# gusanagy/Hybrid-Diffusion-Underwater-Atmopheric-Image-Enhancement

Measured on AMD Instinct MI355X. Metric: denoising-steps/sec (256x256, T=1000), higher is better.
Workload: dtype f32 (tensors and accumulation fp32; every operand of the attention contractions as 2xfp16 pieces -- scores: a balance per product term, four terms at d_head 16 / three at d_head 32; P.V: three terms -- and of the 3x3 convs behind GroupNorm likewise (other 3x3 convs: 3xbf16 pieces), on the 16-bit MFM

## Files before the change

### hybrid-diffusion-underwater-atmopheric-image-enhancement_amd/csrc/attention_x3p.hip

```cpp
#include <stdlib.h>

#include "common.h"
#include "device.h"

using namespace hdiff;

namespace {

constexpr int D = 32;
constexpr int KT = 64;
constexpr int THREADS = 256;
constexpr int NQT = 3;

__global__ __launch_bounds__(THREADS, 2) void mha_flash_fwd_x3p_kernel(const __bf16* __restrict__ ws, float* __restrict__ out,
                                                                      float* __restrict__ lse2, int C, int L, float one) {
  constexpr int KS = D / 16;
  constexpr int KROWB = D * 2 + 16;
  constexpr int KPART = KT * KROWB;
  constexpr int VROWB = KT * 2 + 8;
  constexpr int VPART = D * VROWB;
  constexpr int NKC = NQT * KT * D / 8;
  constexpr int NVC = 2 * D * 8;
  constexpr int NLD = (NKC + NVC) / THREADS;
  static_assert((NKC + NVC) % THREADS == 0, "staging geometry");
  constexpr int QB = 256;
  constexpr int VBASE = NQT * KPART;
  constexpr int BUFB = (VBASE + 2 * VPART + 15) / 16 * 16;
  __shared__ __attribute__((aligned(16))) unsigned char smem[2][BUFB];

  const int tid = threadIdx.x, lane = tid & 63, wave = tid >> 6;
  const int l31 = lane & 31, h = lane >> 5;
  const TileId tile = xcd_tile();
  const int head = tile.head, b = tile.b;
  const int heads = gridDim.y;
  const int qblk0 = tile.x * QB + wave * 64;
  const size_t piece = (size_t)L * D;
  const __bf16* qs = ws + ((size_t)b * heads + head) * F_COUNT * piece;
  const __bf16* ks = qs + F_K * piece;
  const __bf16* vs = qs + F_V * piece;
  const int ntiles = L / KT;

  u32x4 qop[2][NQT][KS];
#pragma unroll
  for (int G = 0; G < 2; ++G) {
    const int q = qblk0 + 32 * G + l31;
#pragma unroll
    for (int p = 0; p < 2; ++p)
#pragma unroll
      for (int s = 0; s < KS; ++s)
        qop[G][p][s] = *reinterpret_cast<const u32x4*>(qs + p * piece + (size_t)q * D + 16 * s + 8 * h);
    const unsigned dn2 = PAIR_DOWN2;
#pragma unroll
    for (int s = 0; s < KS; ++s) {
      unsigned w4[4];
#pragma unroll
      for (int w = 0; w < 4; ++w) asm("v_pk_mul_f16 %0, %1, %2" : "=v"(w4[w]) : "v"(qop[G][0][s][w]), "v"(dn2));
      qop[G][2][s] = u32x4{w4[0], w4[1], w4[2], w4[3]};
    }
  }

  const unsigned char* gsrc[NLD];
  int lds_off[NLD];
  int gstep[NLD];
#pragma unroll
  for (int i = 0; i < NLD; ++i) {
    const int c = i * THREADS + tid;
    if (c < NKC) {
      const int p = c / (KT * D / 8), rem = c - p * (KT * D / 8);
      const int key = rem / (D / 8), part = rem - key * (D / 8);
      gsrc[i] = reinterpret_cast<const unsigned char*>(ks + p * piece) + (size_t)rem * 16;
      lds_off[i] = p * KPART + key * KROWB + part * 16;
      gstep[i] = KT * D * 2;
    } else {
      const int cv = c - NKC;
      const int p = cv / (D * 8), rem = cv - p * (D * 8);
      const int d = rem >> 3, seg = rem & 7;
      gsrc[i] = reinterpret_cast<const unsigned char*>(vs + p * piece + (size_t)d * L) + seg * 16;
      lds_off[i] = VBASE + p * VPART + d * VROWB + seg * 16;
      gstep[i] = KT * 2;
    }
  }
  u32x4 stage[NLD];
  auto stage_load = [&](int t) {
#pragma unroll
    for (int i = 0; i < NLD; ++i) stage[i] = *reinterpret_cast<const u32x4*>(gsrc[i] + (size_t)t * gstep[i]);
  };
  auto stage_store = [&](int buf) {
#pragma unroll
    for (int i = 0; i < NLD; ++i) {
      unsigned char* dst = &smem[buf][lds_off[i]];
      *reinterpret_cast<u32x2*>(dst) = u32x2{stage[i][0], stage[i][1]};
      *reinterpret_cast<u32x2*>(dst + 8) = u32x2{stage[i][2], stage[i][3]};
    }
  };

  const int kaddr = l31 * KROWB + 16 * h;
  int vaddr[2];
#pragma unroll
  for (int p = 0; p < 2; ++p) vaddr[p] = p * VPART + l31 * VROWB + 8 * h;

  f32x16 O[2], negm16;
  f32x2 l_run[2];
  float negm2[2] = {0.f, 0.f};
#pragma unroll
  for (int G = 0; G < 2; ++G) {
    l_run[G] = f32x2{0.f, 0.f};
#pragma unroll
    for (int r = 0; r < 16; ++r) O[G][r] = 0.f;
  }
#pragma unroll
  for (int r = 0; r < 16; ++r) negm16[r] = 0.f;

  auto load_k = [&](int buf, int kb, u32x4 (&kop)[NQT][KS]) {
    const unsigned char* kbuf = smem[buf] + kb * 32 * KROWB + kaddr;
#pragma unroll
    for (int p = 0; p < NQT; ++p)
#pragma unroll
      for (int s = 0; s < KS; ++s) kop[p][s] = *reinterpret_cast<const u32x4*>(kbuf + p * KPART + 32 * s);
  };
  auto load_v = [&](int buf, int kb, u32x4 (&vop)[2][2]) {
    const unsigned char* vbuf = smem[buf] + VBASE + kb * 64;
#pragma unroll
    for (int ab = 0; ab < 2; ++ab)
#pragma unroll
      for (int p = 0; p < 2; ++p) {
        const unsigned char* src = vbuf + vaddr[p] + 32 * ab;
        const u32x2 lo = *reinterpret_cast<const u32x2*>(src);
        const u32x2 hi2 = *reinterpret_cast<const u32x2*>(src + 16);
        vop[ab][p] = u32x4{lo[0], lo[1], hi2[0], hi2[1]};
      }
  };
  auto qk = [&](const u32x4 (&kop)[NQT][KS], int G, f32x16 c) {
    f32x16 S = c;
#pragma unroll
    for (int term = 0; term < NQT; ++term)
#pragma unroll
      for (int s = 0; s < KS; ++s) {
        u32x4 qb = qop[G][term][s];
        if ((HDIFF_MUTANT & 2) && term == 1)
#pragma unroll
          for (int w = 0; w < 4; ++w) qb[w] &= 0xffe0ffe0u;
        S = mfma_f16(kop[term][s], qb, S);
      }
    return S;
  };
  auto exp_pairs = [&](const f32x16& S, u32x4 (&pop)[2][2], float& sum0, float& sum1) {
    sum0 = 0.f; sum1 = 0.f;
#pragma unroll
    for (int j = 0; j < 4; ++j) {
      const float p0 = __builtin_amdgcn_exp2f(S[4 * j]), p1 = __builtin_amdgcn_exp2f(S[4 * j + 1]);
      const float p2 = __builtin_amdgcn_exp2f(S[4 * j + 2]), p3 = __builtin_amdgcn_exp2f(S[4 * j + 3]);
      sum0 += p0 + p2;
      sum1 += p1 + p3;
      unsigned a0, a1, c0, c1;
      split2(p0, p1, one, a0, a1);
      split2(p2, p3, one, c0, c1);
      const int ab = j >> 1, o = (j & 1) * 2;
      pop[ab][0][o] = a0; pop[ab][1][o] = a1;
      pop[ab][0][o + 1] = c0; pop[ab][1][o + 1] = c1;
    }
  };
  auto softmax_pairs = [&](f32x16& S, int G, u32x4 (&pop)[2][2]) {
    float sum0, sum1;
    exp_pairs(S, pop, sum0, sum1);
    if (__builtin_amdgcn_ballot_w64(sum0 + sum1 >= P_TRIP) != 0ull) {
      float mx = fmaxf(fmaxf(S[0], S[1]), fmaxf(S[2], S[3]));
#pragma unroll
      for (int j = 1; j < 4; ++j) mx = fmaxf(mx, fmaxf(fmaxf(S[4 * j], S[4 * j + 1]), fmaxf(S[4 * j + 2], S[4 * j + 3])));
      mx = fmaxf(mx, __shfl_xor(mx, 32, 64));
      const float delta = (mx > P_SHIFT + 1.0f) ? __builtin_ceilf(mx - P_SHIFT) : 0.f;
      const int e = -(int)delta;
#pragma unroll
      for (int r = 0; r < 16; ++r) O[G][r] = __builtin_ldexpf(O[G][r], e);
      l_run[G][0] = __builtin_ldexpf(l_run[G][0], e);
      l_run[G][1] = __builtin_ldexpf(l_run[G][1], e);
      negm2[G] -= delta;
#pragma unroll
      for (int r = 0; r < 16; ++r) S[r] -= delta;
      exp_pairs(S, pop, sum0, sum1);
    }
    l_run[G][0] += sum0;
    l_run[G][1] += sum1;
  };
  auto pv = [&](const u32x4 (&vop)[2][2], const u32x4 (&pop)[2][2], int G) {
#pragma unroll
    for (int ab = 0; ab < 2; ++ab) {
      O[G] = mfma_f16(vop[ab][1], pop[ab][0], O[G]);
      O[G] = mfma_f16(vop[ab][0], pop[ab][1], O[G]);
      O[G] = mfma_f16(vop[ab][0], pop[ab][0], O[G]);
    }
  };

  stage_load(0);
  stage_store(0);
  __syncthreads();
  stage_load(ntiles > 1 ? 1 : 0);
  {
    u32x4 K0[NQT][KS];
    load_k(0, 0, K0);
    const f32x16 s0 = qk(K0, 0, negm16), s1 = qk(K0, 1, negm16);
    float t0 = s0[0], t1 = s1[0];
#pragma unroll
    for (int r = 1; r < 16; ++r) { t0 = fmaxf(t0, s0[r]); t1 = fmaxf(t1, s1[r]); }
    negm2[0] = P_SHIFT - fmaxf(t0, __shfl_xor(t0, 32, 64));
    negm2[1] = P_SHIFT - fmaxf(t1, __shfl_xor(t1, 32, 64));
  }
  auto block = [&](int buf, int kb) {
    u32x4 kop[NQT][KS], vop[2][2];
    load_k(buf, kb, kop);
    load_v(buf, kb, vop);
    f32x16 S2[2];
#pragma unroll
    for (int G = 0; G < 2; ++G) {
      float nm = negm2[G];
      asm volatile("" : "+v"(nm));
#pragma unroll
      for (int r = 0; r < 16; ++r) negm16[r] = nm;
      S2[G] = qk(kop, G, negm16);
    }
#pragma unroll
    for (int G = 0; G < 2; ++G) {
      u32x4 pop[2][2];
      softmax_pairs(S2[G], G, pop);
      pv(vop, pop, G);
    }
  };
  block(0, 0);
  block(0, 1);
  stage_store(1);
  __syncthreads();
  for (int t = 1; t < ntiles; ++t) {
    const int buf = t & 1;
    stage_load((t + 1 < ntiles) ? t + 1 : t);
    block(buf, 0);
    block(buf, 1);
    stage_store(buf ^ 1);
    __syncthreads();
  }

  float* obase = out + ((size_t)b * C + (size_t)head * D) * L;
  const float* vinv = reinterpret_cast<const float*>(qs + 8 * piece);
#pragma unroll
  for (int G = 0; G < 2; ++G) {
    float lt = l_run[G][0] + l_run[G][1];
    lt += __shfl_xor(lt, 32, 64);
    const bool bad = !(lt < OVERFLOW_LIMIT);
    const float inv = bad ? __builtin_nanf("") : 1.0f / lt;
    const int q = qblk0 + 32 * G + l31;
    if (lse2 != nullptr && h == 0)
      lse2[((size_t)b * heads + head) * L + q] = bad ? __builtin_nanf("") : __builtin_amdgcn_logf(lt) - negm2[G];
#pragma unroll
    for (int r = 0; r < 16; ++r) {
      const int d = 8 * (r >> 2) + 4 * h + (r & 3);
      obase[(size_t)d * L + q] = (O[G][r] * inv) * vinv[d];
    }
  }
}

}

namespace hdiff {

int64_t mha_fwd_x3p_workspace(int B, int C, int heads, int L) {
  const int Dh = C / heads;
  if ((Dh != 16 && Dh != 32) || L % 256 != 0 || L < 512) return 0;
  return (int64_t)B * C * L * F_COUNT * 2 + mha_fwd_h2_tail_bytes(B, C);
}

void launch_mha_fwd_x3p(const float* qkv, float* o, float* lse2, int B, int C, int heads, int L, float qscale, void* ws,
                        hipStream_t stream) {
  launch_qk_split_h2(qkv, ws, B, C, heads, L, qscale, stream);
  launch_v_split_h2(qkv, ws, B, C, heads, L, stream);
  hipLaunchKernelGGL(mha_flash_fwd_x3p_kernel, dim3(L / 256, heads, B), dim3(THREADS), 0, stream, (const __bf16*)ws, o, lse2, C, L, 1.0f);
}

}
```

Measured before the change: 2.978.

## Software-pipeline QK/softmax/PV across query groups and DMA K tiles into LDS

The flash-attention kernel now interleaves the QK and PV MFMAs of one query group with the exp/split softmax VALU work of the other, using sched_barrier to pin the interleave. K tiles are loaded straight into LDS with a direct global-to-LDS DMA using an XOR-swizzled layout, replacing the padded register-staged copy. Prefetch moves two tiles ahead with an explicit vmcnt wait. This aims to hide MFMA and VALU latency behind each other and cut staging instructions, at the cost of more register pressure and more complex scheduling.

```diff
diff --git a/hybrid-diffusion-underwater-atmopheric-image-enhancement_amd/csrc/attention_x3p.hip b/hybrid-diffusion-underwater-atmopheric-image-enhancement_amd/csrc/attention_x3p.hip
--- a/hybrid-diffusion-underwater-atmopheric-image-enhancement_amd/csrc/attention_x3p.hip
+++ b/hybrid-diffusion-underwater-atmopheric-image-enhancement_amd/csrc/attention_x3p.hip
@@ -1,4 +1,6 @@
 #include <stdlib.h>
+
+#include <type_traits>
 
 #include "common.h"
 #include "device.h"
@@ -15,14 +17,14 @@
 __global__ __launch_bounds__(THREADS, 2) void mha_flash_fwd_x3p_kernel(const __bf16* __restrict__ ws, float* __restrict__ out,
                                                                       float* __restrict__ lse2, int C, int L, float one) {
   constexpr int KS = D / 16;
-  constexpr int KROWB = D * 2 + 16;
+  constexpr int KROWB = D * 2;
   constexpr int KPART = KT * KROWB;
   constexpr int VROWB = KT * 2 + 8;
   constexpr int VPART = D * VROWB;
-  constexpr int NKC = NQT * KT * D / 8;
   constexpr int NVC = 2 * D * 8;
-  constexpr int NLD = (NKC + NVC) / THREADS;
-  static_assert((NKC + NVC) % THREADS == 0, "staging geometry");
+  constexpr int NLD = NVC / THREADS;
+  static_assert(NVC % THREADS == 0, "staging geometry");
+  static_assert(NQT * KPART == 3 * (THREADS / 64) * 1024, "LDS-DMA geometry: twelve 1 KiB runs, three per wave");
   constexpr int QB = 256;
   constexpr int VBASE = NQT * KPART;
   constexpr int BUFB = (VBASE + 2 * VPART + 15) / 16 * 16;
@@ -59,31 +61,33 @@
     }
   }
 
+  const unsigned kdma_voff = (unsigned)(((lane >> 2) * 4 + ((lane & 3) ^ ((lane >> 4) & 3))) * 16);
+  const unsigned lds0 = (unsigned)(size_t)(lds_byte*)&smem[0][0];
+  const unsigned char* kdma = reinterpret_cast<const unsigned char*>(ks);
+  auto dma_k = [&](int t, int buf) {
+    const int w3 = __builtin_amdgcn_readfirstlane(wave) * 3;
+#pragma unroll
+    for (int i = 0; i < 3; ++i) {
+      const int run = w3 + i, p = run >> 2, quarter = run & 3;
+      const unsigned char* src = kdma + (size_t)p * (piece * 2) + (size_t)t * KPART + quarter * 1024;
+      const unsigned dst = __builtin_amdgcn_readfirstlane(lds0 + buf * BUFB + run * 1024);
+      dma_1k(src, kdma_voff, dst);
+    }
+  };
   const unsigned char* gsrc[NLD];
   int lds_off[NLD];
-  int gstep[NLD];
 #pragma unroll
   for (int i = 0; i < NLD; ++i) {
-    const int c = i * THREADS + tid;
-    if (c < NKC) {
-      const int p = c / (KT * D / 8), rem = c - p * (KT * D / 8);
-      const int key = rem / (D / 8), part = rem - key * (D / 8);
-      gsrc[i] = reinterpret_cast<const unsigned char*>(ks + p * piece) + (size_t)rem * 16;
-      lds_off[i] = p * KPART + key * KROWB + part * 16;
-      gstep[i] = KT * D * 2;
-    } else {
-      const int cv = c - NKC;
-      const int p = cv / (D * 8), rem = cv - p * (D * 8);
-      const int d = rem >> 3, seg = rem & 7;
-      gsrc[i] = reinterpret_cast<const unsigned char*>(vs + p * piece + (size_t)d * L) + seg * 16;
-      lds_off[i] = VBASE + p * VPART + d * VROWB + seg * 16;
-      gstep[i] = KT * 2;
-    }
+    const int cv = i * THREADS + tid;
+    const int p = cv / (D * 8), rem = cv - p * (D * 8);
+    const int d = rem >> 3, seg = rem & 7;
+    gsrc[i] = reinterpret_cast<const unsigned char*>(vs + p * piece + (size_t)d * L) + seg * 16;
+    lds_off[i] = VBASE + p * VPART + d * VROWB + seg * 16;
   }
   u32x4 stage[NLD];
   auto stage_load = [&](int t) {
 #pragma unroll
-    for (int i = 0; i < NLD; ++i) stage[i] = *reinterpret_cast<const u32x4*>(gsrc[i] + (size_t)t * gstep[i]);
+    for (int i = 0; i < NLD; ++i) stage[i] = *reinterpret_cast<const u32x4*>(gsrc[i] + (size_t)t * (KT * 2));
   };
   auto stage_store = [&](int buf) {
 #pragma unroll
@@ -94,31 +98,34 @@
     }
   };
 
-  const int kaddr = l31 * KROWB + 16 * h;
+  int kaddr[KS];
+#pragma unroll
+  for (int s = 0; s < KS; ++s) kaddr[s] = l31 * KROWB + 16 * ((2 * s + h) ^ ((l31 >> 2) & 3));
   int vaddr[2];
 #pragma unroll
   for (int p = 0; p < 2; ++p) vaddr[p] = p * VPART + l31 * VROWB + 8 * h;
 
-  f32x16 O[2], negm16;
+  f32x16 O[2], negm16[2];
   f32x2 l_run[2];
-  float negm2[2] = {0.f, 0.f};
 #pragma unroll
   for (int G = 0; G < 2; ++G) {
     l_run[G] = f32x2{0.f, 0.f};
 #pragma unroll
-    for (int r = 0; r < 16; ++r) O[G][r] = 0.f;
-  }
-#pragma unroll
-  for (int r = 0; r < 16; ++r) negm16[r] = 0.f;
-
-  auto load_k = [&](int buf, int kb, u32x4 (&kop)[NQT][KS]) {
-    const unsigned char* kbuf = smem[buf] + kb * 32 * KROWB + kaddr;
+    for (int r = 0; r < 16; ++r) { O[G][r] = 0.f; negm16[G][r] = 0.f; }
+  }
+
+  u32x4 kop[NQT][KS];
+  u32x4 vop[2][2];
+  f32x16 S[2];
+  u32x4 pop[2][2][2];
+  auto load_k = [&](int buf, int kb) {
+    const unsigned char* kbuf = smem[buf] + kb * 32 * KROWB;
 #pragma unroll
     for (int p = 0; p < NQT; ++p)
 #pragma unroll
-      for (int s = 0; s < KS; ++s) kop[p][s] = *reinterpret_cast<const u32x4*>(kbuf + p * KPART + 32 * s);
-  };
-  auto load_v = [&](int buf, int kb, u32x4 (&vop)[2][2]) {
+      for (int s = 0; s < KS; ++s) kop[p][s] = *reinterpret_cast<const u32x4*>(kbuf + p * KPART + kaddr[s]);
+  };
+  auto load_v = [&](int buf, int kb) {
     const unsigned char* vbuf = smem[buf] + VBASE + kb * 64;
 #pragma unroll
     for (int ab = 0; ab < 2; ++ab)
@@ -130,43 +137,82 @@
         vop[ab][p] = u32x4{lo[0], lo[1], hi2[0], hi2[1]};
       }
   };
-  auto qk = [&](const u32x4 (&kop)[NQT][KS], int G, f32x16 c) {
-    f32x16 S = c;
-#pragma unroll
-    for (int term = 0; term < NQT; ++term)
-#pragma unroll
-      for (int s = 0; s < KS; ++s) {
-        u32x4 qb = qop[G][term][s];
-        if ((HDIFF_MUTANT & 2) && term == 1)
-#pragma unroll
-          for (int w = 0; w < 4; ++w) qb[w] &= 0xffe0ffe0u;
-        S = mfma_f16(kop[term][s], qb, S);
-      }
-    return S;
-  };
-  auto exp_pairs = [&](const f32x16& S, u32x4 (&pop)[2][2], float& sum0, float& sum1) {
-    sum0 = 0.f; sum1 = 0.f;
+  constexpr int NQK = NQT * KS, NPV = 6;
+  auto qk_mfma = [&](int G, int n) {
+    const int term = n / KS, s = n - term * KS;
+    u32x4 qb = qop[G][term][s];
+    if ((HDIFF_MUTANT & 2) && term == 1)
+#pragma unroll
+      for (int w = 0; w < 4; ++w) qb[w] &= 0xffe0ffe0u;
+    S[G] = mfma_f16(kop[term][s], qb, n == 0 ? negm16[G] : S[G]);
+  };
+  auto pv_mfma = [&](int G, int n) {
+    const int ab = n / 3, term = n - ab * 3;
+    O[G] = mfma_f16(vop[ab][term == 0 ? 1 : 0], pop[G][ab][term == 1 ? 1 : 0], O[G]);
+  };
+  auto exp_pairs = [&](const f32x16& Sq, u32x4 (&pp)[2][2], float& sum0, float& sum1) {
 #pragma unroll
     for (int j = 0; j < 4; ++j) {
-      const float p0 = __builtin_amdgcn_exp2f(S[4 * j]), p1 = __builtin_amdgcn_exp2f(S[4 * j + 1]);
-      const float p2 = __builtin_amdgcn_exp2f(S[4 * j + 2]), p3 = __builtin_amdgcn_exp2f(S[4 * j + 3]);
-      sum0 += p0 + p2;
-      sum1 += p1 + p3;
+      const float p0 = __builtin_amdgcn_exp2f(Sq[4 * j]), p1 = __builtin_amdgcn_exp2f(Sq[4 * j + 1]);
+      const float p2 = __builtin_amdgcn_exp2f(Sq[4 * j + 2]), p3 = __builtin_amdgcn_exp2f(Sq[4 * j + 3]);
+      sum0 = (j == 0) ? p0 + p2 : sum0 + (p0 + p2);
+      sum1 = (j == 0) ? p1 + p3 : sum1 + (p1 + p3);
       unsigned a0, a1, c0, c1;
       split2(p0, p1, one, a0, a1);
       split2(p2, p3, one, c0, c1);
       const int ab = j >> 1, o = (j & 1) * 2;
-      pop[ab][0][o] = a0; pop[ab][1][o] = a1;
-      pop[ab][0][o + 1] = c0; pop[ab][1][o + 1] = c1;
-    }
-  };
-  auto softmax_pairs = [&](f32x16& S, int G, u32x4 (&pop)[2][2]) {
+      pp[ab][0][o] = a0; pp[ab][1][o] = a1;
+      pp[ab][0][o + 1] = c0; pp[ab][1][o + 1] = c1;
+    }
+  };
+  auto stage_fn = [&](auto g_tag, auto pend_tag, int kload_buf, int kload_kb, int vload_buf, int vload_kb) __attribute__((always_inline)) {
+    constexpr int G = decltype(g_tag)::value;
+    constexpr bool PEND = decltype(pend_tag)::value;
+    constexpr int NM = NQK + (PEND ? NPV : 0);
+    if (kload_buf >= 0) load_k(kload_buf, kload_kb);
     float sum0, sum1;
-    exp_pairs(S, pop, sum0, sum1);
+    float pe[4][4], ad[4][2];
+    unsigned u[4][2], r2[4][2];
+    _Float16 rl[4][2];
+    auto vstep = [&](int n) {
+      const int j = n / 14, r = n - j * 14;
+      if (r < 4) pe[j][r] = __builtin_amdgcn_exp2f(S[G][4 * j + r]);
+      else if (r < 6) {
+        const f16x2 p = {(_Float16)pe[j][2 * (r - 4)], (_Float16)pe[j][2 * (r - 4) + 1]};
+        unsigned w = __builtin_bit_cast(unsigned, p);
+        asm("" : "+v"(w));
+        u[j][r - 4] = w;
+      } else if (r < 8) ad[j][r - 6] = pe[j][r - 6] + pe[j][r - 6 + 2];
+      else if (r < 10) rl[j][r - 8] = (_Float16)__builtin_fmaf(pe[j][2 * (r - 8)], one, -(float)__builtin_bit_cast(f16x2, u[j][r - 8])[0]);
+      else if (r < 12) {
+        const f16x2 pr = {rl[j][r - 10],
+                          (_Float16)__builtin_fmaf(pe[j][2 * (r - 10) + 1], one, -(float)__builtin_bit_cast(f16x2, u[j][r - 10])[1])};
+        unsigned w = __builtin_bit_cast(unsigned, pr);
+        asm("" : "+v"(w));
+        r2[j][r - 10] = w;
+      } else if (r == 12) sum0 = (j == 0) ? ad[j][0] : sum0 + ad[j][0];
+      else sum1 = (j == 0) ? ad[j][1] : sum1 + ad[j][1];
+    };
+    constexpr int NV = 56;
+#pragma unroll
+    for (int i = 0; i < NM; ++i) {
+      if (PEND && i < NPV) pv_mfma(G ^ 1, i);
+      else qk_mfma(G ^ 1, i - (PEND ? NPV : 0));
+      if (PEND && i == NPV - 1 && vload_buf >= 0) load_v(vload_buf, vload_kb);
+#pragma unroll
+      for (int n = NV * i / NM; n < NV * (i + 1) / NM; ++n) vstep(n);
+      __builtin_amdgcn_sched_barrier(0);
+    }
+#pragma unroll
+    for (int j = 0; j < 4; ++j) {
+      const int ab = j >> 1, o = (j & 1) * 2;
+      pop[G][ab][0][o] = u[j][0]; pop[G][ab][1][o] = r2[j][0];
+      pop[G][ab][0][o + 1] = u[j][1]; pop[G][ab][1][o + 1] = r2[j][1];
+    }
     if (__builtin_amdgcn_ballot_w64(sum0 + sum1 >= P_TRIP) != 0ull) {
-      float mx = fmaxf(fmaxf(S[0], S[1]), fmaxf(S[2], S[3]));
-#pragma unroll
-      for (int j = 1; j < 4; ++j) mx = fmaxf(mx, fmaxf(fmaxf(S[4 * j], S[4 * j + 1]), fmaxf(S[4 * j + 2], S[4 * j + 3])));
+      float mx = fmaxf(fmaxf(S[G][0], S[G][1]), fmaxf(S[G][2], S[G][3]));
+#pragma unroll
+      for (int j = 1; j < 4; ++j) mx = fmaxf(mx, fmaxf(fmaxf(S[G][4 * j], S[G][4 * j + 1]), fmaxf(S[G][4 * j + 2], S[G][4 * j + 3])));
       mx = fmaxf(mx, __shfl_xor(mx, 32, 64));
       const float delta = (mx > P_SHIFT + 1.0f) ? __builtin_ceilf(mx - P_SHIFT) : 0.f;
       const int e = -(int)delta;
@@ -174,69 +220,57 @@
       for (int r = 0; r < 16; ++r) O[G][r] = __builtin_ldexpf(O[G][r], e);
       l_run[G][0] = __builtin_ldexpf(l_run[G][0], e);
       l_run[G][1] = __builtin_ldexpf(l_run[G][1], e);
-      negm2[G] -= delta;
-#pragma unroll
-      for (int r = 0; r < 16; ++r) S[r] -= delta;
-      exp_pairs(S, pop, sum0, sum1);
+#pragma unroll
+      for (int r = 0; r < 16; ++r) { negm16[G][r] -= delta; S[G][r] -= delta; }
+      exp_pairs(S[G], pop[G], sum0, sum1);
     }
     l_run[G][0] += sum0;
     l_run[G][1] += sum1;
   };
-  auto pv = [&](const u32x4 (&vop)[2][2], const u32x4 (&pop)[2][2], int G) {
-#pragma unroll
-    for (int ab = 0; ab < 2; ++ab) {
-      O[G] = mfma_f16(vop[ab][1], pop[ab][0], O[G]);
-      O[G] = mfma_f16(vop[ab][0], pop[ab][1], O[G]);
-      O[G] = mfma_f16(vop[ab][0], pop[ab][0], O[G]);
-    }
-  };
-
+  using G0 = std::integral_constant<int, 0>;
+  using G1 = std::integral_constant<int, 1>;
+  auto tile_fn = [&](auto first_tag, int t) __attribute__((always_inline)) {
+    constexpr bool FIRST = decltype(first_tag)::value;
+    using Pend = std::integral_constant<bool, !FIRST>;
+    const int buf = t & 1;
+    stage_fn(G0{}, Pend{}, -1, 0, FIRST ? -1 : buf, 0);
+    stage_fn(G1{}, std::true_type{}, buf, 1, -1, 0);
+    stage_fn(G0{}, std::true_type{}, -1, 0, buf, 1);
+    stage_store(buf ^ 1);
+    asm volatile("s_waitcnt vmcnt(0)" ::: "memory");
+    __syncthreads();
+    const int tn = (t + 2 < ntiles) ? t + 2 : ntiles - 1;
+    dma_k(tn, buf);
+    stage_load(tn);
+    stage_fn(G1{}, std::true_type{}, buf ^ 1, 0, -1, 0);
+  };
+
+  dma_k(0, 0);
   stage_load(0);
   stage_store(0);
+  asm volatile("s_waitcnt vmcnt(0)" ::: "memory");
   __syncthreads();
+  dma_k(ntiles > 1 ? 1 : 0, 1);
   stage_load(ntiles > 1 ? 1 : 0);
+  load_k(0, 0);
   {
-    u32x4 K0[NQT][KS];
-    load_k(0, 0, K0);
-    const f32x16 s0 = qk(K0, 0, negm16), s1 = qk(K0, 1, negm16);
-    float t0 = s0[0], t1 = s1[0];
-#pragma unroll
-    for (int r = 1; r < 16; ++r) { t0 = fmaxf(t0, s0[r]); t1 = fmaxf(t1, s1[r]); }
-    negm2[0] = P_SHIFT - fmaxf(t0, __shfl_xor(t0, 32, 64));
-    negm2[1] = P_SHIFT - fmaxf(t1, __shfl_xor(t1, 32, 64));
-  }
-  auto block = [&](int buf, int kb) {
-    u32x4 kop[NQT][KS], vop[2][2];
-    load_k(buf, kb, kop);
-    load_v(buf, kb, vop);
-    f32x16 S2[2];
-#pragma unroll
-    for (int G = 0; G < 2; ++G) {
-      float nm = negm2[G];
-      asm volatile("" : "+v"(nm));
-#pragma unroll
-      for (int r = 0; r < 16; ++r) negm16[r] = nm;
-      S2[G] = qk(kop, G, negm16);
-    }
-#pragma unroll
-    for (int G = 0; G < 2; ++G) {
-      u32x4 pop[2][2];
-      softmax_pairs(S2[G], G, pop);
-      pv(vop, pop, G);
-    }
-  };
-  block(0, 0);
-  block(0, 1);
-  stage_store(1);
-  __syncthreads();
-  for (int t = 1; t < ntiles; ++t) {
-    const int buf = t & 1;
-    stage_load((t + 1 < ntiles) ? t + 1 : t);
-    block(buf, 0);
-    block(buf, 1);
-    stage_store(buf ^ 1);
-    __syncthreads();
-  }
+#pragma unroll
+    for (int n = 0; n < NQK; ++n) { qk_mfma(0, n); qk_mfma(1, n); }
+    float t0 = S[0][0], t1 = S[1][0];
+#pragma unroll
+    for (int r = 1; r < 16; ++r) { t0 = fmaxf(t0, S[0][r]); t1 = fmaxf(t1, S[1][r]); }
+    const float nm0 = P_SHIFT - fmaxf(t0, __shfl_xor(t0, 32, 64)), nm1 = P_SHIFT - fmaxf(t1, __shfl_xor(t1, 32, 64));
+#pragma unroll
+    for (int r = 0; r < 16; ++r) { negm16[0][r] = nm0; negm16[1][r] = nm1; }
+  }
+  load_v(0, 0);
+#pragma unroll
+  for (int n = 0; n < NQK; ++n) qk_mfma(0, n);
+  tile_fn(std::true_type{}, 0);
+  for (int t = 1; t < ntiles; ++t) tile_fn(std::false_type{}, t);
+#pragma unroll
+  for (int n = 0; n < NPV; ++n) pv_mfma(1, n);
+  asm volatile("s_waitcnt vmcnt(0)" ::: "memory");
 
   float* obase = out + ((size_t)b * C + (size_t)head * D) * L;
   const float* vinv = reinterpret_cast<const float*>(qs + 8 * piece);
@@ -248,7 +282,7 @@
     const float inv = bad ? __builtin_nanf("") : 1.0f / lt;
     const int q = qblk0 + 32 * G + l31;
     if (lse2 != nullptr && h == 0)
-      lse2[((size_t)b * heads + head) * L + q] = bad ? __builtin_nanf("") : __builtin_amdgcn_logf(lt) - negm2[G];
+      lse2[((size_t)b * heads + head) * L + q] = bad ? __builtin_nanf("") : __builtin_amdgcn_logf(lt) - negm16[G][0];
 #pragma unroll
     for (int r = 0; r < 16; ++r) {
       const int d = 8 * (r >> 2) + 4 * h + (r & 3);
```

New measurement: 3.003 (median of 6 runs). No clear change (+0.9%).
